# kehanxuuu/vspg-pbrt-v4

Hardware: AMD Instinct MI355X
Metric: Mpaths/sec on 1920x1080 homogeneous fog; relMSE vs CPU ref at equal spp (higher is better)
Workload: dtype f32; 1 GPU; fog-box 1920x1080, guidedvolpathvspg vspguiding=true (primary-ray VSP; App. F options), 1 spp per step per GPU, independent sampler seed 0, maxdepth 5

## Files before the change

### vspg-pbrt-v4_amd/csrc/vspg_capi.hip

```cpp
#include <hip/hip_runtime.h>
#include <dlfcn.h>

#include <cmath>
#include <cstdio>
#include <cstdlib>
#include <cstring>
#include <string>
#include <type_traits>
#include <vector>
#include <algorithm>

#include "vspg_path.h"
#include "vspg_wg_kernel.h"
#include "vspg_guided_wg.h"
#include "vspg_wg3.h"
#include "vspg_trace.h"
#include "vspg_wavefront.h"
#include "vspg_wf_launch.h"
#include "vspg_film_error.h"
#include "vspg_film_resolve.h"
#include "vspg_kernel_choice.h"
#ifdef VSPG_SINGLE_TU
#include "vspg_wf_grid.hip"
#include "vspg_wf_nvdb.hip"
// ... 1880 lines not shown
            float kd = in.Kd[k];
            kd = kd < 0 ? 0 : (kd > 1 ? 1 : kd);
            q.Kd[k] = kd;
            q.Le[k] = in.Le[k];
            lobes = lobes || kd != 0;
            light = light || in.Le[k] != 0;
        }
        q.two_sided = in.two_sided;
        q.is_light = light;
        q.has_lobes = lobes;
        q.flags = surf_flags_of(in.material, in.medium_interface);
        auto single_axis = [](const float *v) {
            int nz = 0, ax = -1;
            for (int k = 0; k < 3; ++k)
                if (v[k] != 0) { nz++; ax = k; }
            return nz == 1 ? ax : -1;
        };
        int an = single_axis(q.n), a1 = single_axis(q.e1), a2 = single_axis(q.e2);
        IsectRec &rec = D->irec[i];
        memset(&rec, 0, sizeof rec);
        if (an >= 0 && a1 >= 0 && a2 >= 0 && an != a1 && an != a2 && a1 != a2 && std::fabs(q.n[an]) == 1.0f) {
            rec.kind = 1;
            rec.axes = an | (a1 << 2) | (a2 << 4);
            rec.f[0] = q.n[an]; rec.f[1] = q.p00[an]; rec.f[2] = q.p00[a1]; rec.f[3] = q.p00[a2];
            rec.f[4] = q.e1[a1]; rec.f[5] = q.e2[a2]; rec.f[6] = q.inv_l1; rec.f[7] = q.inv_l2;
        } else {
            rec.kind = 0;
            for (int k = 0; k < 3; ++k) { rec.f[k] = q.n[k]; rec.f[3 + k] = q.p00[k]; rec.f[6 + k] = q.e1[k]; rec.f[9 + k] = q.e2[k]; }
            rec.f[12] = q.inv_l1; rec.f[13] = q.inv_l2;
        }
        if (light) D->light_quads[D->n_lights++] = i;
    }
    D->n_inf = sc.n_infinite_lights;
    for (int i = 0; i < sc.n_infinite_lights && i < VSPG_MAX_INFINITE_LIGHTS; ++i) {
        D->inf_type[i] = sc.infinite_lights[i].type;
        for (int k = 0; k < 3; ++k) { D->inf_L[i][k] = sc.infinite_lights[i].L[k]; D->inf_w[i][k] = sc.infinite_lights[i].w_light[k]; }
    }
    {
        float lo[3] = {kInf, kInf, kInf}, hi[3] = {-kInf, -kInf, -kInf};
        auto grow = [&](const float *q) { for (int k = 0; k < 3; ++k) { lo[k] = q[k] < lo[k] ? q[k] : lo[k]; hi[k] = q[k] > hi[k] ? q[k] : hi[k]; } };
        for (int i = 0; i < D->n_quads; ++i) { grow(D->quads[i].p00); grow(D->quads[i].p10); grow(D->quads[i].p01); grow(D->quads[i].p11); }
        for (int i = 0; i < sc.n_triangles && sc.tri_p; ++i) {
            DTri T;
            if (derive_triangle(sc.tri_p + 9 * (size_t)i, nullptr, i, &T)) { grow(T.p0); grow(T.p1); grow(T.p2); }
        }
        for (int i = 0; i < sc.n_spheres; ++i) {
            const float *m = sc.spheres[i].render_from_object, rr = sc.spheres[i].radius;
            for (int c = 0; c < 8; ++c) {
// ... 1979 lines not shown
```

### vspg-pbrt-v4_amd/csrc/vspg_device.h

```cpp
#pragma once
#include <hip/hip_runtime.h>
#include <stdint.h>

#include "../../include/vspg.h"
#include "vspg_arith.h"
#include "vspg_libm.h"

#define VDEV __device__ __forceinline__
#ifdef VSPG_WF_DEBUG
__device__ unsigned int g_dbg_err[8];
#define VSPG_DBG_CHECK(cond, bit) do { if (!(cond)) atomicOr(&g_dbg_err[0], 1u << (bit)); } while (0)
#else
#define VSPG_DBG_CHECK(cond, bit)
#endif
#ifdef VSPG_NOINLINE_LEAVES
#define VLEAF __device__ __attribute__((noinline))
#else
#define VLEAF __device__ __forceinline__
#endif

VSPG_NS_BEGIN

#ifdef VSPG_PROFILE
enum { PS_INTERSECT = 0, PS_HASHRNG, PS_DIST_GUIDED, PS_DIST_PLAIN, PS_SURF_PRE, PS_NEE, PS_NEE_TR, PS_VOL_SAMPLE,
// ... 403 lines not shown
    uint32_t r = ui + ((uint32_t)((int32_t)(ui ^ os) >> 31) | 1u);
    r = (ui << 1) == 0u ? (os | 1u) : r;
    const bool keep = !__builtin_islessgreater(off, 0.f) || (ui ^ os) == 0x7f800000u;
    return b2f(keep ? ui : r);
}
VDEV V3 offset_ray_origin(P3i pi, V3 n, V3 w) {
    float d = dot(vabs(n), pi.err());
    V3 offset = n * d;
    if (dot(w, n) < 0) offset = -offset;
    V3 po = pi.mid() + offset;
    return V3{offset_axis(po.x, offset.x), offset_axis(po.y, offset.y), offset_axis(po.z, offset.z)};
}

#define VSPG_GLOBAL_AS __attribute__((address_space(1)))
struct DQuad {
    float p00[3], p10[3], p01[3], p11[3], e1[3], e2[3];
    float n[3], dpdu_n[3], perr[3];
    float inv_l1, inv_l2, area;
    float Kd[3], Le[3];
    int32_t two_sided, is_light, has_lobes;
    int32_t flags;
};
enum { SURF_INTERFACE = 1, SURF_IFACE_SHIFT = 1 };
struct IsectRec {
    float f[14];
    int32_t kind;
    int32_t axes;
};
struct DField {
    int32_t n_nodes, n_regions;
    const VspgKdNode *nodes;
    const VspgFieldRegion *regions;
    const float *aux;
    const float4 *lobes;
};
constexpr int kMaxLights = VSPG_MAX_QUADS + VSPG_MAX_INFINITE_LIGHTS;
struct DLightNode {
    float bmin[3], bmax[3], w[3];
    float phi, cosTheta_o, cosTheta_e;
    int32_t twoSided;
    uint32_t child_or_light;
    int32_t is_leaf;
};
struct DLightSampler {
    int32_t mode;
    int32_t n_nodes, n_inf, n_alias;
    DLightNode nodes[2 * kMaxLights];
    int32_t inf_light[VSPG_MAX_INFINITE_LIGHTS];
    uint32_t bit_trail[kMaxLights];
    float alias_p[kMaxLights], alias_q[kMaxLights];
    int32_t alias_i[kMaxLights];
// ... 101 lines not shown
                            : k < 13 ? S.sigma_t[k - 10] : S.sigma_n_raw[k - 13];
    }
}
VDEV const DQuad &quad_at(int i) { return s_scene_quads[i]; }
VDEV const DQuad &light_quad_at(int lightIndex) { return s_scene_quads[s_scene_light_quads[lightIndex]]; }

struct Isect {
    bool hit;
    float t;
    int quad;
    V3 p, n;
};
VDEV bool is_tri(int prim) { return prim <= -2; }
VDEV int tri_of(int prim) { return -2 - prim; }
constexpr int kSpherePrim = 32;
static_assert(VSPG_MAX_QUADS <= kSpherePrim, "rectangle indices lie below the first sphere primitive");
VDEV bool is_sphere(int prim) { return prim >= kSpherePrim; }
VDEV int sphere_of(int prim) { return prim - kSpherePrim; }

VDEV bool beyond(float num, float denom, float tMax) {
    return __builtin_fabsf(num) > tMax * __builtin_fabsf(denom) * 1.000001f;
}
VDEV float comp(V3 v, int axis) { return axis == 0 ? v.x : (axis == 1 ? v.y : v.z); }
VDEV bool rect_hit_uv(const IsectRec &r, V3 o, V3 d, float tMax, float *tHit, float *uHit, float *vHit) {
    float num, denom, u, v, t;
    if (r.kind == 1) {
        const int a = r.axes & 3, ua = (r.axes >> 2) & 3, va = (r.axes >> 4) & 3;
        denom = r.f[0] * comp(d, a);
        num = r.f[0] * (r.f[1] - comp(o, a));
        bool cand = (num > 0 && denom > 0) || (num < 0 && denom < 0);
        if (!cand) return false;
        if (beyond(num, denom, tMax)) return false;
        t = num / denom;
        if (!(t > 0) || !(t < tMax)) return false;
        float pu = comp(o, ua) + comp(d, ua) * t, pv = comp(o, va) + comp(d, va) * t;
        u = ((pu - r.f[2]) * r.f[4]) * r.f[6];
        v = ((pv - r.f[3]) * r.f[5]) * r.f[7];
    } else {
        V3 n = V3{r.f[0], r.f[1], r.f[2]}, p00 = V3{r.f[3], r.f[4], r.f[5]};
        denom = dot(n, d);
        num = dot(n, p00 - o);
        bool cand = (num > 0 && denom > 0) || (num < 0 && denom < 0);
        if (!cand) return false;
        if (beyond(num, denom, tMax)) return false;
        t = num / denom;
        if (!(t > 0) || !(t < tMax)) return false;
        V3 p = o + d * t;
        V3 rel = p - p00;
        u = dot(rel, V3{r.f[6], r.f[7], r.f[8]}) * r.f[12];
        v = dot(rel, V3{r.f[9], r.f[10], r.f[11]}) * r.f[13];
    }
    if (u < 0 || u > 1 || v < 0 || v > 1) return false;
    *tHit = t;
    *uHit = u;
    *vHit = v;
    return true;
}
VDEV bool quad_hit_uv(const DQuad &q, V3 o, V3 d, float tMax, float *tHit, float *uHit, float *vHit) {
    V3 n = ld3(q.n), p00 = ld3(q.p00);
    float denom = dot(n, d);
    float num = dot(n, p00 - o);
    bool cand = (num > 0 && denom > 0) || (num < 0 && denom < 0);
    if (!cand) return false;
    float t = num / denom;
    if (!(t > 0) || !(t < tMax)) return false;
    V3 p = o + d * t;
    V3 rel = p - p00;
    float u = dot(rel, ld3(q.e1)) * q.inv_l1;
    float v = dot(rel, ld3(q.e2)) * q.inv_l2;
    if (u < 0 || u > 1 || v < 0 || v > 1) return false;
    *tHit = t;
    *uHit = u;
    *vHit = v;
// ... 251 lines not shown
        pv[k] = (row[0] * x + row[1] * y) + (row[2] * z + row[3]);
        const float ea = g3 * (__builtin_fabsf(row[0] * x) + __builtin_fabsf(row[1] * y) + __builtin_fabsf(row[2] * z) + __builtin_fabsf(row[3]));
        pe[k] = exact ? ea : (g3 + 1) * (__builtin_fabsf(row[0]) * ex + __builtin_fabsf(row[1]) * ey + __builtin_fabsf(row[2]) * ez) + ea;
    }
    r.pi = p3i_from_err(V3{pv[0], pv[1], pv[2]}, V3{pe[0], pe[1], pe[2]});
    const float *mi = S.mi;
    r.n = normalize(V3{mi[0] * no.x + mi[4] * no.y + mi[8] * no.z, mi[1] * no.x + mi[5] * no.y + mi[9] * no.z, mi[2] * no.x + mi[6] * no.y + mi[10] * no.z});
    if (WITH_DPDU) {
        const float *m = S.m;
        r.dpdu_n = normalize(V3{m[0] * dpdu.x + m[1] * dpdu.y + m[2] * dpdu.z, m[4] * dpdu.x + m[5] * dpdu.y + m[6] * dpdu.z, m[8] * dpdu.x + m[9] * dpdu.y + m[10] * dpdu.z});
    } else {
        r.dpdu_n = mk(0, 0, 0);
    }
    return r;
}

template <bool FULL = true>
VLEAF Isect scene_intersect(const DScene &S, V3 o, V3 d, float tMax) {
    Isect best;
    best.hit = false;
    best.t = tMax;
    best.quad = 0;
    float bu = 0, bv = 0;
    for (int i = 0; i < S.n_quads; ++i) {
        float t, u, v;
        if (rect_hit_uv(S.irec[i], o, d, best.t, &t, &u, &v)) {
            best.hit = true;
            best.t = t;
            best.quad = i;
            bu = u;
            bv = v;
        }
    }
    const DQuad &q = quad_at(best.quad);
    best.p = quad_point(q, bu, bv);
    best.n = ld3(q.n);
    if (FULL && S.n_tris > 0) {
        int tp = 0;
        TriHit h;
        if (bvh_closest(S, o, d, best.t, &tp, &h)) {
            const DTri &T = S.tris[tp];
            best.hit = true;
            best.t = h.t;
            best.quad = -2 - tp;
            best.p = V3{h.b0, h.b1, h.b2};
            best.n = V3{T.nx, T.ny, T.nz};
        }
    }
    if (FULL && S.n_spheres > 0) {
        for (int i = 0; i < S.n_spheres; ++i) {
            float t;
            V3 pObj;
            if (sphere_intersect(S.spheres[i], o, d, tMax, &t, &pObj) && t < best.t) {
                best.hit = true;
                best.t = t;
                best.quad = kSpherePrim + i;
                best.p = pObj;
                best.n = sphere_interaction<false>(S.spheres[i], pObj).n;
            }
        }
    }
    return best;
}
template <bool FULL = true>
VLEAF bool scene_intersect_any(const DScene &S, V3 o, V3 d, float tMax) {
    bool any = false;
    for (int i = 0; i < S.n_quads; ++i) {
        float t, u, v;
        any = any || rect_hit_uv(S.irec[i], o, d, tMax, &t, &u, &v);
    }
    if (FULL && S.n_tris > 0 && !any) any = bvh_any(S, o, d, tMax);
    if (FULL && S.n_spheres > 0 && !any) {
        for (int i = 0; i < S.n_spheres; ++i) {
            float t;
            V3 pObj;
            any = any || sphere_intersect(S.spheres[i], o, d, tMax, &t, &pObj);
        }
    }
    return any;
}
VDEV int surf_flags(const DScene &S, int prim) {
    if (is_tri(prim)) return S.tris[tri_of(prim)].flags;
    if (is_sphere(prim)) return S.spheres[sphere_of(prim)].flags;
    return quad_at(prim).flags;
}
VDEV P3i tri_pi(const DTri &T, V3 b) {
    const V3 p0 = ld3(T.p0), p1 = ld3(T.p1), p2 = ld3(T.p2);
    const V3 p = p0 * b.x + p1 * b.y + p2 * b.z;
    const V3 s = vabs(p0 * b.x) + vabs(p1 * b.y) + vabs(p2 * b.z);
    constexpr float g7 = (7 * kMachineEps) / (1 - 7 * kMachineEps);
    return p3i_from_err(p, V3{g7 * s.x, g7 * s.y, g7 * s.z});
}
// ... 647 lines not shown
```

### vspg-pbrt-v4_amd/csrc/vspg_wg3.h

```cpp
#pragma once
#include <type_traits>

#include "vspg_guided_wg.h"
#include "vspg_path.h"
#include "vspg_wg_kernel.h"

VSPG_NS_BEGIN

enum { Q_VV = 0, Q_VS = 1, Q_A = 2, Q_F = 3, Q_COUNT = 4 };
enum { QC_RES = 0, QC_COM = 1, QC_HEAD = 2, QC_STRIDE = 4 };
enum { W3_BUSY_S = Q_COUNT * QC_STRIDE, W3_BUSY_V, W3_EXH, W3_LIVE, W3_COUNT };
enum { W3_OLD = Q_VV * QC_STRIDE + 3, W3_SUSP_LO = Q_VS * QC_STRIDE + 3, W3_SUSP_HI = Q_A * QC_STRIDE + 3 };
constexpr unsigned kCarryDrainBit = 0x80000000u;
enum { W3_NONE = 0, W3_VERTEX = 1, W3_SEGMENT = 2, W3_FRESH = 3, W3_EXIT = 4 };
constexpr unsigned kRestartBit = 0x8000u;

VDEV float isg_code(const IsgSample &isg) {
    if (!isg.valid) return 0.f;
    const float q = isg.vsp_used >= 0.f ? isg.vsp_used : 0.5f;
    return isg.surface_event ? -q : q;
}
__device__ __forceinline__ void resolve_sample(float4 s, float4 *film_px, float *isg_px) {
    const Spec L = Spec{s.x, s.y, s.z};
    film_add_sample_rmw(film_px, L);
    IsgSample isg;
    isg.valid = s.w != 0.f;
    isg.surface_event = s.w < 0.f;
    isg.vsp_used = __builtin_fabsf(s.w);
    isg_add_sample_rmw(isg_px, L, isg);
}
template <class T>
__device__ __forceinline__ T w3_at_use(T v) {
    asm volatile("" : "+s"(v));
    return v;
}
__device__ __forceinline__ int w3_lane() {
    int l = (int)(threadIdx.x & 63u);
    asm volatile("" : "+v"(l));
    return l;
}
constexpr float kCarrySentinel = 2.f;
__device__ __forceinline__ bool carry_sentinel(float w) { return w > 1.f; }
template <class LY, int NP> constexpr int kWg3ImagePool = LY::COUNT * NP;
template <class LY, int NP> constexpr int kWg3ImageWords = LY::COUNT * NP + Q_COUNT * NP / 2;
template <class LY, int NP> constexpr int kWg3ImageStride = kWg3ImageWords<LY, NP> + 32;
static_assert(W3_COUNT <= 32, "the image's queue words");

constexpr int kWg3Heads = 8, kWg3HeadSetBytes = kWg3Heads * 128;
__device__ __forceinline__ void reset_sibling_head(unsigned int *work_head) {
    if (blockIdx.x == 0 && threadIdx.x == 0) *reinterpret_cast<unsigned int *>(reinterpret_cast<uintptr_t>(work_head) ^ 4u) = 0u;
}

typedef unsigned int w3_u32x4 __attribute__((ext_vector_type(4)));
typedef const volatile __attribute__((address_space(3))) w3_u32x4 *w3_lds_v4;
template <int NP>
VDEV void ring_push_all(int dq, unsigned entry, unsigned short (*ring)[NP], unsigned int *s_w) {
    const int lane = w3_lane();
    const unsigned long long m0 = __ballot(dq == 0), m1 = __ballot(dq == 1), m2 = __ballot(dq == 2), m3 = __ballot(dq == 3);
    const unsigned n0 = (unsigned)__popcll(m0), n1 = (unsigned)__popcll(m1), n2 = (unsigned)__popcll(m2), n3 = (unsigned)__popcll(m3);
    const unsigned myn = lane == 0 ? n0 : lane == 1 ? n1 : lane == 2 ? n2 : n3;
    unsigned base = 0;
    if (lane < Q_COUNT && myn > 0u) base = atomicAdd(s_w + lane * QC_STRIDE + QC_RES, myn);
    const unsigned b0 = (unsigned)__builtin_amdgcn_readlane((int)base, 0), b1 = (unsigned)__builtin_amdgcn_readlane((int)base, 1);
// ... 31 lines not shown
struct W3Timeline {
    unsigned long long *rec, t0;
    unsigned phase;
    __device__ __forceinline__ bool mine() const { return (threadIdx.x & 63u) == 0u && blockIdx.x < (unsigned)W3T_MAX_BLOCKS; }
    __device__ __forceinline__ W3Timeline() : rec(&g_w3_timeline[blockIdx.x % W3T_MAX_BLOCKS][(threadIdx.x >> 6) & 7u][0]), t0(0), phase(0) { stamp(W3T_BEGIN); }
    __device__ __forceinline__ void stamp(int i) { const unsigned long long t = __builtin_amdgcn_s_memrealtime(); if (mine()) rec[i] = t; }
    __device__ __forceinline__ void enter(unsigned p, int i) { if (phase < p) { phase = p; stamp(i); } }
    __device__ __forceinline__ void chunk_begin() { t0 = __builtin_amdgcn_s_memrealtime(); }
    __device__ __forceinline__ void chunk_end(unsigned kind, unsigned lanes) {
        const unsigned long long t1 = __builtin_amdgcn_s_memrealtime();
        if (mine()) {
            unsigned long long *r = rec + W3T_SUMS + (phase * 3u + kind) * 3u;
            atomicAdd(r, 1ull); atomicAdd(r + 1, (unsigned long long)lanes); atomicAdd(r + 2, t1 - t0);
        }
    }
};
#define VSPG_W3T(x) x
#else
#define VSPG_W3T(x)
#endif

template <class Medium, bool GUIDED, int NP, int kWgBlock, int kWgWavesPerSimd, bool TRAIN, bool WINDOW, bool CARRY = false>
__device__ __forceinline__ void wg3_render(
    const DScene *__restrict__ Sp, float4 *__restrict__ film, float *__restrict__ isg_stats, const float *__restrict__ vsp_buf,
    int vsp_ready, int wave_end, int first_sample, int single_sample, PcgJump jump, unsigned int tiles_magic,
    unsigned int *__restrict__ work_head, const float4 *__restrict__ prev_samples,
    float4 *__restrict__ wave_samples, unsigned long long *__restrict__ counters, TrainArgs train, const PixelWindow win,
    const unsigned int *__restrict__ resume = nullptr, unsigned int *__restrict__ suspend = nullptr) {
    static_assert(!CARRY || (!TRAIN && !GUIDED), "CARRY serves the unguided one-sample launches");
    vsp_ready = w3_at_use(vsp_ready), wave_end = w3_at_use(wave_end), first_sample = w3_at_use(first_sample);
    single_sample = w3_at_use(single_sample);
    const DScene &S = *Sp;
    const int W = S.xres, H = S.yres;
    const int tilesX = WINDOW ? win_tiles_x(win) : (W + 7) >> 3, tilesY = WINDOW ? win_tiles_y(win) : (H + 7) >> 3;
    const unsigned n_tiles = CARRY && w3_at_use(suspend) == nullptr ? 0u : (unsigned)(tilesX * tilesY);
    const auto in_launch = [&](int px, int py) {
        if constexpr (WINDOW) return win_has(win, px, py);
        else return px < W && py < H;
    };
    const int lane = threadIdx.x & 63;
    const int sample_step = S.shard_count > 1 ? S.shard_count : 1;
    if (blockIdx.x == 0 && threadIdx.x < (unsigned)kWg3Heads)
        reinterpret_cast<unsigned int *>(reinterpret_cast<uintptr_t>(work_head) ^ (uintptr_t)kWg3HeadSetBytes)[threadIdx.x * 32u] = 0u;
    unsigned wseg = blockIdx.x % (unsigned)kWg3Heads, wtried = 0u;

    constexpr bool FULL = !Medium::kSimpleScene;
    static_assert(!FULL || !GUIDED, "the workgroup kernel's guided vertex (vspg_guided_wg.h) is built for rectangle scenes");
    static_assert(NP < (int)kRestartBit, "a ring entry is the slot plus the restart bit");
    using LY = PoolLayout<GUIDED, Medium::kGrey, TRAIN, FULL>;
    constexpr int NF = LY::COUNT;
    static_assert(!TRAIN || GUIDED, "segment recording belongs to the guided instantiations");
    static_assert(Medium::kSingleSegment, "k_render_wave_wg3 serves homogeneous media (grid media: the wavefront pipeline)");
    __shared__ float s_pool[NF * NP];
    __shared__ unsigned short s_ring[Q_COUNT][NP];
    __shared__ __attribute__((aligned(16))) unsigned int s_w[W3_COUNT];
    const Pool P{s_pool, NP};
    const Medium medium = MediumMaker<Medium>::make(S, nullptr);
    float *glds = nullptr;
    if constexpr (GUIDED && kKdLdsNodes > 0) {
        __shared__ VspgKdNode s_kd[2][kKdLdsNodes > 0 ? kKdLdsNodes : 1];
        for (int f = 0; f < 2; ++f) {
            const int nl = S.field[f].n_nodes < kKdLdsNodes ? S.field[f].n_nodes : kKdLdsNodes;
            for (int i = threadIdx.x; i < nl; i += kWgBlock) s_kd[f][i] = S.field[f].nodes[i];
        }
        glds = reinterpret_cast<float *>(&s_kd[0][0]);
    }
    __shared__ unsigned int s_counters[CNT_COUNT];
    struct LaneCounters : PathCounters { uint32_t paths; VDEV void path() { paths++; } };
    using Rec = typename std::conditional<TRAIN, PathRecorder, NullRecorder>::type;
    typename std::conditional<GUIDED, WaveCountersT<Rec>, LaneCounters>::type pc = [&] {
        if constexpr (GUIDED) { WaveCountersT<Rec> c; c.c = s_counters; return c; }
        else { LaneCounters c; c.segments = c.volume_scatters = c.surface_hits = c.density_queries = c.shadow_rays = c.shadow_queries = c.paths = 0; return c; }
    }();
    const auto rec_bind = [&](int pxy) {
        if constexpr (TRAIN) {
            const unsigned px = (unsigned)pxy & 0xffffu, py = (unsigned)pxy >> 16;
            const unsigned tcol = WINDOW ? (px >> 3) - (unsigned)win_tile_x0(win) : px >> 3, trow = WINDOW ? (py >> 3) - (unsigned)win_tile_y0(win) : py >> 3;
            const unsigned item = (trow * (unsigned)tilesX + tcol) * 64u + ((py & 7u) << 3) + (px & 7u);
            pc.rec.base = train.segbuf + item;
            pc.rec.stride = (int)train.n_items;
            pc.rec.max_seg = train_rec_capacity(S.prm.maxdepth);
            return item;
        } else {
            (void)pxy;
            return 0u;
        }
    };

    stage_scene_lds(S);
    if (threadIdx.x < CNT_COUNT) s_counters[threadIdx.x] = 0;
    constexpr int kImgPool = kWg3ImagePool<LY, NP>, kImgWords = kWg3ImageWords<LY, NP>, kImgStride = kWg3ImageStride<LY, NP>;
    bool resumed = false;
    if constexpr (CARRY) {
        const unsigned int *const img = resume + (size_t)blockIdx.x * kImgStride;
        resumed = resume != nullptr && img[kImgWords + W3_LIVE] != 0u;
        if (resumed) {
            unsigned int *const pool32 = reinterpret_cast<unsigned int *>(s_pool);
#pragma unroll 8
            for (int i = threadIdx.x; i < kImgPool; i += kWgBlock) pool32[i] = img[i];
            unsigned short *const ring16 = &s_ring[0][0];
#pragma unroll 3
            for (int i = threadIdx.x; i < Q_COUNT * NP / 2; i += kWgBlock) {
                const unsigned v = img[kImgPool + i];
                ring16[2 * i] = (unsigned short)(v & 0xffffu);
                ring16[2 * i + 1] = (unsigned short)(v >> 16);
            }
            if (threadIdx.x < W3_COUNT) s_w[threadIdx.x] = img[kImgWords + threadIdx.x];
            __syncthreads();
            if (threadIdx.x < Q_COUNT) {
                const unsigned h = s_w[threadIdx.x * QC_STRIDE + QC_HEAD], n = s_w[threadIdx.x * QC_STRIDE + QC_COM] - h, h2 = h % (unsigned)NP;
                s_w[threadIdx.x * QC_STRIDE + QC_HEAD] = h2;
                s_w[threadIdx.x * QC_STRIDE + QC_RES] = h2 + n;
                s_w[threadIdx.x * QC_STRIDE + QC_COM] = h2 + n;
            }
            if (threadIdx.x == 0) {
                s_w[W3_OLD] = s_w[W3_LIVE];
                s_w[W3_EXH] = 0u;
                s_w[W3_BUSY_S] = 0u;
                s_w[W3_BUSY_V] = 0u;
            }
        }
    }
    if (!resumed) {
        if (threadIdx.x < W3_COUNT) s_w[threadIdx.x] = 0;
        for (int i = threadIdx.x; i < NP; i += kWgBlock) s_ring[Q_F][i] = (unsigned short)i;
        __syncthreads();
        if (threadIdx.x == 0) {
            s_w[Q_F * QC_STRIDE + QC_RES] = NP; s_w[Q_F * QC_STRIDE + QC_COM] = NP;
        }
    }
    if constexpr (CARRY) {
        __syncthreads();
        if (threadIdx.x == 0) {
            if (suspend == nullptr) { s_w[W3_EXH] = 1u; s_w[W3_OLD] |= kCarryDrainBit; }
            s_w[W3_SUSP_LO] = (unsigned)reinterpret_cast<uintptr_t>(suspend);
            s_w[W3_SUSP_HI] = (unsigned)(reinterpret_cast<uintptr_t>(suspend) >> 32);
        }
    }
    __syncthreads();

    auto emit = [&](int pxy, Spec Lraw, const IsgSample &isg, bool old) {
        const Spec L = finish_radiance(Lraw);
        const size_t pidx = (size_t)((unsigned)pxy >> 16) * W + (pxy & 0xffff);
        if (CARRY && old && w3_at_use(first_sample) >= 0) {
            resolve_sample(make_float4(L.r, L.g, L.b, isg_code(isg)), film + pidx, isg_stats + pidx * VSPG_ISG_STATS);
        } else if (w3_at_use(single_sample)) {
            wave_samples[pidx] = make_float4(L.r, L.g, L.b, isg_code(isg));
        } else {
            film_add_sample(film + pidx, L);
            isg_add_sample_atomic(isg_stats + pidx * VSPG_ISG_STATS, L, isg);
        }
    };

    VSPG_PROF(PS_WG_TOTAL);
    VSPG_PROF_ACC(prof_decide, PS_WG_R);
    VSPG_PROF_ACC(prof_idle, PS_WG_BAR_A);
    unsigned idle_polls = 0;
    VSPG_W3T(W3Timeline tl);
    while (true) {
        VSPG_PROF_ACC_BEGIN(prof_decide);
        VSPG_PROF_ACC_BEGIN(prof_idle);
        unsigned kind = W3_NONE, pos0 = 0, n0 = 0, pos1 = 0, n1 = 0, q0 = Q_VV, tile = 0;
        unsigned fresh_entry = 0;
        {
            const auto U = [](unsigned v) { return (unsigned)__builtin_amdgcn_readfirstlane((int)v); };
            const w3_lds_v4 qw = (w3_lds_v4)(s_w);
            const w3_u32x4 wVV = qw[Q_VV], wVS = qw[Q_VS], wA = qw[Q_A], wF = qw[Q_F], wM = qw[Q_COUNT];
            const unsigned hVV = U(wVV.z), hVS = U(wVS.z), hA = U(wA.z), hF = U(wF.z);
            const unsigned busyS = U(wM.x), busyV = U(wM.y), live = U(wM.w);
            const unsigned old_word = CARRY ? U(wVV.w) : 1u;
            const bool exh = U(wM.z) != 0u;
            VSPG_W3T(if (exh) tl.enter(2u, W3T_EXH));
            const auto avail = [&](w3_u32x4 q, unsigned head) {
// ... 18 lines not shown
                } else {
                    bump(W3_BUSY_V, -1);
                }
            };
            const auto claim_segment = [&]() {
                bump(W3_BUSY_S, 1);
                const unsigned na = (unsigned)(aA < 64 ? aA : 64);
                if (claim(Q_A, hA, na)) { kind = W3_SEGMENT; pos0 = hA; n0 = na; }
                else bump(W3_BUSY_S, -1);
            };
            const int aV = aVV + aVS;
            if (CARRY && exh && old_word == 0u) kind = W3_EXIT;
            else if (aVV >= 64) claim_vertex(aVV, hVV, Q_VV, 0, hVS, Q_VS);
            else if (aVS >= 64) claim_vertex(aVS, hVS, Q_VS, 0, hVV, Q_VV);
            else if (aA >= 64) claim_segment();
            else if (aF >= 64) {
                bump(W3_BUSY_S, 1);
                bump(W3_LIVE, 64);
                if (claim(Q_F, hF, 64u)) {
                    kind = W3_FRESH; pos0 = hF; n0 = 64u;
                    __builtin_amdgcn_fence(__ATOMIC_ACQUIRE, "workgroup");
                    fresh_entry = s_ring[Q_F][(hF + (unsigned)lane) % (unsigned)NP];
                    tile = n_tiles;
                    while (wtried < (unsigned)kWg3Heads) {
                        unsigned c = 0xffffffffu;
                        if (w3_lane() == 0 && __hip_atomic_load(work_head + wseg * 32u, __ATOMIC_RELAXED, __HIP_MEMORY_SCOPE_AGENT) * (unsigned)kWg3Heads + wseg < n_tiles)
                            c = atomicAdd(work_head + wseg * 32u, 1u);
                        c = U(c);
                        if (c != 0xffffffffu && c * (unsigned)kWg3Heads + wseg < n_tiles) {
                            tile = c * (unsigned)kWg3Heads + wseg;
                            break;
                        }
                        wseg = (wseg + 1u) % (unsigned)kWg3Heads;
                        ++wtried;
                    }
                } else {
                    bump(W3_LIVE, -64);
                    bump(W3_BUSY_S, -1);
                }
            } else if (aV >= 64 || (aV > 0 && busyS == 0u)) {
                if (aVV >= aVS) claim_vertex(aVV, hVV, Q_VV, aVS, hVS, Q_VS);
                else claim_vertex(aVS, hVS, Q_VS, aVV, hVV, Q_VV);
            } else if (aA > 0 && busyV == 0u) {
                claim_segment();
            } else if (exh && live == 0u) {
                kind = W3_EXIT;
// ... 76 lines not shown
                freed = true;
            } else if ((unsigned)lane < n0) {
                const unsigned e = fresh ? fresh_entry : s_ring[Q_A][(pos0 + (unsigned)lane) % (unsigned)NP];
                slot = (int)(e & (kRestartBit - 1u));
                const bool primary = fresh || (e & kRestartBit) != 0u;
                Sampler sampler;
                PathState st;
                IsgSample isg;
                int ch = 0, pxy = 0;
                Vertex vx;
                bool alive = false, valid = true;
                int seg = LI_END;
                if (primary) {
                    int px, py, smp;
                    if (fresh) {
                        unsigned ty = w3_at_use(tilesX) == 1 ? tile : __umulhi(tile, tiles_magic);
                        unsigned tx = tile - ty * (unsigned)tilesX;
                        while (tx >= (unsigned)tilesX) { tx -= (unsigned)tilesX; ty++; }
                        if constexpr (WINDOW) { tx += (unsigned)win_tile_x0(win); ty += (unsigned)win_tile_y0(win); }
                        px = (int)(tx * 8u + ((unsigned)lane & 7u));
                        py = (int)(ty * 8u + ((unsigned)lane >> 3));
                        pxy = px | (py << 16);
                        smp = first_sample;
                        if (w3_at_use(prev_samples) != nullptr && in_launch(px, py)) {
                            const size_t pidx = (size_t)py * W + px;
                            const float4 parked = prev_samples[pidx];
                            if (!(CARRY && carry_sentinel(parked.w)))
                                resolve_sample(parked, film + pidx, isg_stats + pidx * VSPG_ISG_STATS);
                        }
                    } else {
                        pxy = P.i(LY::PIXEL, slot);
                        smp = P.i(LY::SAMPLE, slot);
                        px = pxy & 0xffff;
                        py = (int)((unsigned)pxy >> 16);
                    }
                    valid = in_launch(px, py) && smp < wave_end;
                    if (valid) {
                        if (w3_at_use(single_sample))
                            start_path(S, vsp_buf, w3_at_use(vsp_ready), px, py, jump, sampler, st, &ch, isg);
                        else
                            start_path(S, vsp_buf, w3_at_use(vsp_ready), px, py, smp, sampler, st, &ch, isg);
                        P.i(LY::PIXEL, slot) = pxy;
                        P.i(LY::SAMPLE, slot) = smp;
                        if constexpr (TRAIN) { (void)rec_bind(pxy); pc.rec.reset(); }
                        seg = li_segment_a<Medium, GUIDED, SEG_PRIMARY>(S, medium, vsp_buf, w3_at_use(vsp_ready), px, py, st, ch, sampler,
                                                                        isg, pc, vx);
                        alive = seg != LI_END;
                        if (alive) {
                            pool_store_full<GUIDED, Medium::kGrey, FULL>(P, slot, st, sampler, ch, isg, FL_LIVE | (seg == LI_VERTEX && vx.volume ? (uint32_t)FL_VX_VOLUME : 0u));
                            if (seg == LI_VERTEX) pool_store_vertex<GUIDED, Medium::kGrey>(P, slot, vx);
                            if constexpr (TRAIN) pool_store_rec<LY>(P, slot, pc.rec);
// ... 32 lines not shown
                    freed = !restart;
                }
            }
            ring_push_all<NP>(toVV ? Q_VV : toVS ? Q_VS : (toA || restart) ? Q_A : (freed ? Q_F : -1), (unsigned)slot | (restart ? kRestartBit : 0u), s_ring, s_w);
            const unsigned n_freed = (unsigned)__popcll(__ballot(freed));
            const unsigned n_old = CARRY ? (unsigned)__popcll(__ballot(old_done)) : 0u;
            if (w3_lane() == 0) {
                if (CARRY && n_old) atomicSub(s_w + W3_OLD, n_old);
                if (fresh && !tile_ok) atomicExch(s_w + W3_EXH, 1u);
                if (n_freed) atomicSub(s_w + W3_LIVE, n_freed);
                atomicSub(s_w + W3_BUSY_S, 1u);
            }
            VSPG_W3T(tl.chunk_end(fresh ? 2u : 1u, tile_ok ? n0 : 0u));
        }
    }
    VSPG_W3T(tl.stamp(W3T_EXIT));
    if constexpr (!GUIDED) {
        atomicAdd(&s_counters[CNT_PATHS], pc.paths); atomicAdd(&s_counters[CNT_SEGMENTS], pc.segments);
        atomicAdd(&s_counters[CNT_VOLUME_SCATTERS], pc.volume_scatters); atomicAdd(&s_counters[CNT_SURFACE_HITS], pc.surface_hits);
        atomicAdd(&s_counters[CNT_DENSITY_QUERIES], pc.density_queries); atomicAdd(&s_counters[CNT_SHADOW_RAYS], pc.shadow_rays);
        atomicAdd(&s_counters[CNT_SHADOW_QUERIES], pc.shadow_queries);
    }
    __syncthreads();
    if (threadIdx.x < CNT_COUNT) atomicAdd(&counters[threadIdx.x], (unsigned long long)s_counters[threadIdx.x]);
    if constexpr (CARRY) {
        unsigned int *const susp = reinterpret_cast<unsigned int *>((uintptr_t)s_w[W3_SUSP_LO] | ((uintptr_t)s_w[W3_SUSP_HI] << 32));
        if (susp != nullptr) {
            unsigned int *const img = susp + (size_t)blockIdx.x * kImgStride;
            if (threadIdx.x < W3_COUNT) img[kImgWords + threadIdx.x] = s_w[threadIdx.x];
            if (s_w[W3_LIVE] != 0u) {
                const unsigned int *const pool32 = reinterpret_cast<const unsigned int *>(s_pool);
                for (int i = threadIdx.x; i < kImgPool; i += kWgBlock) img[i] = pool32[i];
                const unsigned short *const ring16 = &s_ring[0][0];
                for (int i = threadIdx.x; i < Q_COUNT * NP / 2; i += kWgBlock) img[kImgPool + i] = (unsigned)ring16[2 * i] | ((unsigned)ring16[2 * i + 1] << 16);
                for (int q = 0; q < Q_F; ++q) {
                    const unsigned h = s_w[q * QC_STRIDE + QC_HEAD], n = s_w[q * QC_STRIDE + QC_COM] - h;
                    for (unsigned i = threadIdx.x; i < n && i < (unsigned)NP; i += kWgBlock) {
                        const int pxy = P.i(LY::PIXEL, (int)(s_ring[q][(h + i) % (unsigned)NP] & (kRestartBit - 1u)) % NP);
                        const unsigned px = (unsigned)pxy & 0xffffu, py = (unsigned)pxy >> 16;
                        if (in_launch((int)px, (int)py)) wave_samples[(size_t)py * W + px].w = kCarrySentinel;
                    }
                }
            }
        }
    }
}

template <class Medium, bool GUIDED, int NP, int kWgBlock, int kWgWavesPerSimd, bool TRAIN = false>
__global__ __launch_bounds__(kWgBlock, kWgWavesPerSimd) void k_render_wave_wg3(
    const DScene *__restrict__ Sp, float4 *__restrict__ film, float *__restrict__ isg_stats, const float *__restrict__ vsp_buf,
    int vsp_ready, int wave_end, int first_sample, int single_sample, PcgJump jump, unsigned int tiles_magic,
    unsigned int *__restrict__ work_head, const float4 *__restrict__ prev_samples,
    float4 *__restrict__ wave_samples, unsigned long long *__restrict__ counters, TrainArgs train = TrainArgs{nullptr, nullptr, nullptr, nullptr, 0, 0}) {
    wg3_render<Medium, GUIDED, NP, kWgBlock, kWgWavesPerSimd, TRAIN, false>(Sp, film, isg_stats, vsp_buf, vsp_ready, wave_end, first_sample, single_sample, jump,
                                                                            tiles_magic, work_head, prev_samples, wave_samples, counters, train, PixelWindow{0, 0, 0, 0});
}
template <class Medium, bool GUIDED, int NP, int kWgBlock, int kWgWavesPerSimd, bool TRAIN = false>
__global__ __launch_bounds__(kWgBlock, kWgWavesPerSimd) void k_render_wave_wg3_window(
    const DScene *__restrict__ Sp, float4 *__restrict__ film, float *__restrict__ isg_stats, const float *__restrict__ vsp_buf,
    int vsp_ready, int wave_end, int first_sample, int single_sample, PcgJump jump, unsigned int tiles_magic,
    unsigned int *__restrict__ work_head, const float4 *__restrict__ prev_samples,
    float4 *__restrict__ wave_samples, unsigned long long *__restrict__ counters, TrainArgs train, PixelWindow win) {
    wg3_render<Medium, GUIDED, NP, kWgBlock, kWgWavesPerSimd, TRAIN, true>(Sp, film, isg_stats, vsp_buf, vsp_ready, wave_end, first_sample, single_sample, jump,
                                                                           tiles_magic, work_head, prev_samples, wave_samples, counters, train, win);
}

template <class Medium, bool GUIDED, int NP, int kWgBlock, int kWgWavesPerSimd, bool WINDOW>
__global__ __launch_bounds__(kWgBlock, kWgWavesPerSimd) void k_render_wave_wg3_carry(
    const DScene *__restrict__ Sp, float4 *__restrict__ film, float *__restrict__ isg_stats, const float *__restrict__ vsp_buf,
    int vsp_ready, int wave_end, int first_sample, int single_sample, PcgJump jump, unsigned int tiles_magic,
    unsigned int *__restrict__ work_head, const float4 *__restrict__ prev_samples,
    float4 *__restrict__ wave_samples, unsigned long long *__restrict__ counters, PixelWindow win,
    const unsigned int *__restrict__ resume, unsigned int *__restrict__ suspend) {
    wg3_render<Medium, GUIDED, NP, kWgBlock, kWgWavesPerSimd, false, WINDOW, true>(Sp, film, isg_stats, vsp_buf, vsp_ready, wave_end, first_sample, single_sample, jump,
                                                                                   tiles_magic, work_head, prev_samples, wave_samples, counters,
                                                                                   TrainArgs{nullptr, nullptr, nullptr, nullptr, 0, 0}, win, resume, suspend);
}

#ifndef VSPG_WG_WAVES
#define VSPG_WG_WAVES 4
#endif
#ifndef VSPG_WG_BLOCK
#define VSPG_WG_BLOCK 512
#endif
struct Wg3Launch {
    const DScene *dscene;
    float4 *film;
    float *isg_stats;
    const float *vsp;
    int vsp_ready, wave_end, first_sample, single_sample;
    PcgJump jump;
    unsigned int tiles_magic;
    unsigned int *work_head;
    const float4 *ws_prev;
    float4 *ws_out;
    unsigned long long *counters;
    unsigned int blocks;
    hipStream_t stream;
// ... 44 lines not shown
```

Before: 3630 Mpaths/s.

## Split intersection records into 32-byte halves, prefetch heads, reload kernargs at use

Reorders IsectRec into a 32-byte head {kind, axes, f[0..5]} and a 32-byte tail, loaded as 8-wide scalar vectors. The next rectangle's head is prefetched while the current one is tested, and the tail is fetched only once the plane test passes. Separately, kernel pointers (film, isg_stats, wave_samples, counters, prev_samples, work_head) are re-read from the kernarg segment where they are used instead of being held live, to reduce SGPR pressure. The ring load/store becomes 32-bit copies instead of split 16-bit writes. The risks are extra scalar loads and reliance on inline-asm tricks to steer codegen.

```diff
diff --git a/vspg-pbrt-v4_amd/csrc/vspg_capi.hip b/vspg-pbrt-v4_amd/csrc/vspg_capi.hip
--- a/vspg-pbrt-v4_amd/csrc/vspg_capi.hip
+++ b/vspg-pbrt-v4_amd/csrc/vspg_capi.hip
@@ -1926,8 +1926,9 @@
         if (an >= 0 && a1 >= 0 && a2 >= 0 && an != a1 && an != a2 && a1 != a2 && std::fabs(q.n[an]) == 1.0f) {
             rec.kind = 1;
             rec.axes = an | (a1 << 2) | (a2 << 4);
-            rec.f[0] = q.n[an]; rec.f[1] = q.p00[an]; rec.f[2] = q.p00[a1]; rec.f[3] = q.p00[a2];
-            rec.f[4] = q.e1[a1]; rec.f[5] = q.e2[a2]; rec.f[6] = q.inv_l1; rec.f[7] = q.inv_l2;
+            rec.f[0] = q.n[an]; rec.f[1] = q.p00[an];
+            rec.f[6] = q.p00[a1]; rec.f[7] = q.p00[a2];
+            rec.f[8] = q.e1[a1]; rec.f[9] = q.e2[a2]; rec.f[10] = q.inv_l1; rec.f[11] = q.inv_l2;
         } else {
             rec.kind = 0;
             for (int k = 0; k < 3; ++k) { rec.f[k] = q.n[k]; rec.f[3 + k] = q.p00[k]; rec.f[6 + k] = q.e1[k]; rec.f[9 + k] = q.e2[k]; }
diff --git a/vspg-pbrt-v4_amd/csrc/vspg_device.h b/vspg-pbrt-v4_amd/csrc/vspg_device.h
--- a/vspg-pbrt-v4_amd/csrc/vspg_device.h
+++ b/vspg-pbrt-v4_amd/csrc/vspg_device.h
@@ -449,11 +449,16 @@
     int32_t flags;
 };
 enum { SURF_INTERFACE = 1, SURF_IFACE_SHIFT = 1 };
-struct IsectRec {
-    float f[14];
+struct alignas(32) IsectRec {
     int32_t kind;
     int32_t axes;
-};
+    float f[14];
+};
+static_assert(sizeof(IsectRec) == 64 && alignof(IsectRec) == 32, "two 32-byte halves");
+static_assert(offsetof(IsectRec, kind) == 0 && offsetof(IsectRec, axes) == 4 && offsetof(IsectRec, f) == 8, "the head: {kind, axes, f[0..5]}");
+static_assert(offsetof(IsectRec, f) + 6 * sizeof(float) == 32, "the tail f[6..13] is the second half");
+typedef int32_t irec_i32x8 __attribute__((ext_vector_type(8)));
+typedef float irec_f32x8 __attribute__((ext_vector_type(8)));
 struct DField {
     int32_t n_nodes, n_regions;
     const VspgKdNode *nodes;
@@ -601,22 +606,37 @@
     return __builtin_fabsf(num) > tMax * __builtin_fabsf(denom) * 1.000001f;
 }
 VDEV float comp(V3 v, int axis) { return axis == 0 ? v.x : (axis == 1 ? v.y : v.z); }
-VDEV bool rect_hit_uv(const IsectRec &r, V3 o, V3 d, float tMax, float *tHit, float *uHit, float *vHit) {
+template <class T>
+VDEV T rect_half(const DScene &S, int i, uint32_t half) {
+    uint32_t off = (uint32_t)offsetof(DScene, irec) + (uint32_t)i * (uint32_t)sizeof(IsectRec) + half * 32u;
+    asm volatile("" : "+s"(off));
+    return *reinterpret_cast<const T *>(reinterpret_cast<const char *>(&S) + off);
+}
+VDEV irec_i32x8 rect_head(const DScene &S, int i) { return rect_half<irec_i32x8>(S, i, 0u); }
+VDEV irec_f32x8 rect_tail(const DScene &S, int i) { return rect_half<irec_f32x8>(S, i, 1u); }
+VDEV void rect_head_arrived(const irec_i32x8 h) {
+    const int32_t kind = h[0];
+    asm volatile("" : : "s"(kind));
+}
+VDEV bool rect_hit_uv(const DScene &S, int i, const irec_i32x8 h, V3 o, V3 d, float tMax, float *tHit, float *uHit, float *vHit) {
     float num, denom, u, v, t;
-    if (r.kind == 1) {
-        const int a = r.axes & 3, ua = (r.axes >> 2) & 3, va = (r.axes >> 4) & 3;
-        denom = r.f[0] * comp(d, a);
-        num = r.f[0] * (r.f[1] - comp(o, a));
+    const auto hf = [&](int k) { const int32_t w = h[2 + k]; return __builtin_bit_cast(float, w); };
+    if (h[0] == 1) {
+        const int axes = h[1];
+        const int a = axes & 3, ua = (axes >> 2) & 3, va = (axes >> 4) & 3;
+        denom = hf(0) * comp(d, a);
+        num = hf(0) * (hf(1) - comp(o, a));
         bool cand = (num > 0 && denom > 0) || (num < 0 && denom < 0);
         if (!cand) return false;
         if (beyond(num, denom, tMax)) return false;
         t = num / denom;
         if (!(t > 0) || !(t < tMax)) return false;
         float pu = comp(o, ua) + comp(d, ua) * t, pv = comp(o, va) + comp(d, va) * t;
-        u = ((pu - r.f[2]) * r.f[4]) * r.f[6];
-        v = ((pv - r.f[3]) * r.f[5]) * r.f[7];
+        const irec_f32x8 g = rect_tail(S, i);
+        u = ((pu - g[0]) * g[2]) * g[4];
+        v = ((pv - g[1]) * g[3]) * g[5];
     } else {
-        V3 n = V3{r.f[0], r.f[1], r.f[2]}, p00 = V3{r.f[3], r.f[4], r.f[5]};
+        V3 n = V3{hf(0), hf(1), hf(2)}, p00 = V3{hf(3), hf(4), hf(5)};
         denom = dot(n, d);
         num = dot(n, p00 - o);
         bool cand = (num > 0 && denom > 0) || (num < 0 && denom < 0);
@@ -626,8 +646,9 @@
         if (!(t > 0) || !(t < tMax)) return false;
         V3 p = o + d * t;
         V3 rel = p - p00;
-        u = dot(rel, V3{r.f[6], r.f[7], r.f[8]}) * r.f[12];
-        v = dot(rel, V3{r.f[9], r.f[10], r.f[11]}) * r.f[13];
+        const irec_f32x8 g = rect_tail(S, i);
+        u = dot(rel, V3{g[0], g[1], g[2]}) * g[6];
+        v = dot(rel, V3{g[3], g[4], g[5]}) * g[7];
     }
     if (u < 0 || u > 1 || v < 0 || v > 1) return false;
     *tHit = t;
@@ -925,9 +946,14 @@
     best.t = tMax;
     best.quad = 0;
     float bu = 0, bv = 0;
-    for (int i = 0; i < S.n_quads; ++i) {
+    const int nq = S.n_quads;
+    irec_i32x8 head = rect_head(S, 0);
+    for (int i = 0; i < nq; ++i) {
         float t, u, v;
-        if (rect_hit_uv(S.irec[i], o, d, best.t, &t, &u, &v)) {
+        const irec_i32x8 h = head;
+        rect_head_arrived(h);
+        head = rect_head(S, i + 1 < nq ? i + 1 : i);
+        if (rect_hit_uv(S, i, h, o, d, best.t, &t, &u, &v)) {
             best.hit = true;
             best.t = t;
             best.quad = i;
@@ -968,9 +994,14 @@
 template <bool FULL = true>
 VLEAF bool scene_intersect_any(const DScene &S, V3 o, V3 d, float tMax) {
     bool any = false;
-    for (int i = 0; i < S.n_quads; ++i) {
+    const int nq = S.n_quads;
+    irec_i32x8 head = rect_head(S, 0);
+    for (int i = 0; i < nq; ++i) {
         float t, u, v;
-        any = any || rect_hit_uv(S.irec[i], o, d, tMax, &t, &u, &v);
+        const irec_i32x8 h = head;
+        rect_head_arrived(h);
+        head = rect_head(S, i + 1 < nq ? i + 1 : i);
+        any = any || rect_hit_uv(S, i, h, o, d, tMax, &t, &u, &v);
     }
     if (FULL && S.n_tris > 0 && !any) any = bvh_any(S, o, d, tMax);
     if (FULL && S.n_spheres > 0 && !any) {
diff --git a/vspg-pbrt-v4_amd/csrc/vspg_wg3.h b/vspg-pbrt-v4_amd/csrc/vspg_wg3.h
--- a/vspg-pbrt-v4_amd/csrc/vspg_wg3.h
+++ b/vspg-pbrt-v4_amd/csrc/vspg_wg3.h
@@ -39,6 +39,38 @@
     asm volatile("" : "+v"(l));
     return l;
 }
+struct Wg3KernArgs {
+    const DScene *Sp;
+    float4 *film;
+    float *isg_stats;
+    const float *vsp_buf;
+    int vsp_ready, wave_end, first_sample, single_sample;
+    PcgJump jump;
+    unsigned int tiles_magic;
+    unsigned int *work_head;
+    const float4 *prev_samples;
+    float4 *wave_samples;
+    unsigned long long *counters;
+};
+template <class T>
+__device__ __forceinline__ T w3_karg(uint32_t offset) {
+    asm volatile("" : "+s"(offset));
+    typedef const __attribute__((address_space(4))) char *karg_bytes;
+    typedef const __attribute__((address_space(4))) T *karg_T;
+    return *(karg_T)((karg_bytes)__builtin_amdgcn_kernarg_segment_ptr() + offset);
+}
+#define VSPG_W3_KARG(field) w3_karg<decltype(Wg3KernArgs::field)>((uint32_t)offsetof(Wg3KernArgs, field))
+struct Wg3FilmArgs {
+    float4 *film;
+    float *isg_stats;
+};
+static_assert(offsetof(Wg3KernArgs, isg_stats) == offsetof(Wg3KernArgs, film) + sizeof(float4 *) && sizeof(Wg3FilmArgs) == 16, "neighbours");
+typedef unsigned long long w3_u64x2 __attribute__((ext_vector_type(2), aligned(8)));
+__device__ __forceinline__ Wg3FilmArgs w3_film_args() {
+    const w3_u64x2 v = w3_karg<w3_u64x2>((uint32_t)offsetof(Wg3KernArgs, film));
+    return Wg3FilmArgs{reinterpret_cast<float4 *>(v.x), reinterpret_cast<float *>(v.y)};
+}
+
 constexpr float kCarrySentinel = 2.f;
 __device__ __forceinline__ bool carry_sentinel(float w) { return w > 1.f; }
 template <class LY, int NP> constexpr int kWg3ImagePool = LY::COUNT * NP;
@@ -116,10 +148,9 @@
 
 template <class Medium, bool GUIDED, int NP, int kWgBlock, int kWgWavesPerSimd, bool TRAIN, bool WINDOW, bool CARRY = false>
 __device__ __forceinline__ void wg3_render(
-    const DScene *__restrict__ Sp, float4 *__restrict__ film, float *__restrict__ isg_stats, const float *__restrict__ vsp_buf,
+    const DScene *__restrict__ Sp, const float *__restrict__ vsp_buf,
     int vsp_ready, int wave_end, int first_sample, int single_sample, PcgJump jump, unsigned int tiles_magic,
-    unsigned int *__restrict__ work_head, const float4 *__restrict__ prev_samples,
-    float4 *__restrict__ wave_samples, unsigned long long *__restrict__ counters, TrainArgs train, const PixelWindow win,
+    unsigned int *__restrict__ work_head, TrainArgs train, const PixelWindow win,
     const unsigned int *__restrict__ resume = nullptr, unsigned int *__restrict__ suspend = nullptr) {
     static_assert(!CARRY || (!TRAIN && !GUIDED), "CARRY serves the unguided one-sample launches");
     vsp_ready = w3_at_use(vsp_ready), wave_end = w3_at_use(wave_end), first_sample = w3_at_use(first_sample);
@@ -146,7 +177,7 @@
     static_assert(!TRAIN || GUIDED, "segment recording belongs to the guided instantiations");
     static_assert(Medium::kSingleSegment, "k_render_wave_wg3 serves homogeneous media (grid media: the wavefront pipeline)");
     __shared__ float s_pool[NF * NP];
-    __shared__ unsigned short s_ring[Q_COUNT][NP];
+    __shared__ __attribute__((aligned(4))) unsigned short s_ring[Q_COUNT][NP];
     __shared__ __attribute__((aligned(16))) unsigned int s_w[W3_COUNT];
     const Pool P{s_pool, NP};
     const Medium medium = MediumMaker<Medium>::make(S, nullptr);
@@ -192,13 +223,9 @@
             unsigned int *const pool32 = reinterpret_cast<unsigned int *>(s_pool);
 #pragma unroll 8
             for (int i = threadIdx.x; i < kImgPool; i += kWgBlock) pool32[i] = img[i];
-            unsigned short *const ring16 = &s_ring[0][0];
+            unsigned int *const ring32 = reinterpret_cast<unsigned int *>(&s_ring[0][0]);
 #pragma unroll 3
-            for (int i = threadIdx.x; i < Q_COUNT * NP / 2; i += kWgBlock) {
-                const unsigned v = img[kImgPool + i];
-                ring16[2 * i] = (unsigned short)(v & 0xffffu);
-                ring16[2 * i + 1] = (unsigned short)(v >> 16);
-            }
+            for (int i = threadIdx.x; i < Q_COUNT * NP / 2; i += kWgBlock) ring32[i] = img[kImgPool + i];
             if (threadIdx.x < W3_COUNT) s_w[threadIdx.x] = img[kImgWords + threadIdx.x];
             __syncthreads();
             if (threadIdx.x < Q_COUNT) {
@@ -235,14 +262,16 @@
 
     auto emit = [&](int pxy, Spec Lraw, const IsgSample &isg, bool old) {
         const Spec L = finish_radiance(Lraw);
-        const size_t pidx = (size_t)((unsigned)pxy >> 16) * W + (pxy & 0xffff);
+                const size_t pidx = (size_t)((unsigned)pxy >> 16) * W + (pxy & 0xffff);
         if (CARRY && old && w3_at_use(first_sample) >= 0) {
-            resolve_sample(make_float4(L.r, L.g, L.b, isg_code(isg)), film + pidx, isg_stats + pidx * VSPG_ISG_STATS);
+            const Wg3FilmArgs fa = w3_film_args();
+            resolve_sample(make_float4(L.r, L.g, L.b, isg_code(isg)), fa.film + pidx, fa.isg_stats + pidx * VSPG_ISG_STATS);
         } else if (w3_at_use(single_sample)) {
-            wave_samples[pidx] = make_float4(L.r, L.g, L.b, isg_code(isg));
+            VSPG_W3_KARG(wave_samples)[pidx] = make_float4(L.r, L.g, L.b, isg_code(isg));
         } else {
-            film_add_sample(film + pidx, L);
-            isg_add_sample_atomic(isg_stats + pidx * VSPG_ISG_STATS, L, isg);
+            const Wg3FilmArgs fa = w3_film_args();
+            film_add_sample(fa.film + pidx, L);
+            isg_add_sample_atomic(fa.isg_stats + pidx * VSPG_ISG_STATS, L, isg);
         }
     };
 
@@ -307,6 +336,7 @@
                     __builtin_amdgcn_fence(__ATOMIC_ACQUIRE, "workgroup");
                     fresh_entry = s_ring[Q_F][(hF + (unsigned)lane) % (unsigned)NP];
                     tile = n_tiles;
+                    unsigned int *const work_head = VSPG_W3_KARG(work_head);
                     while (wtried < (unsigned)kWg3Heads) {
                         unsigned c = 0xffffffffu;
                         if (w3_lane() == 0 && __hip_atomic_load(work_head + wseg * 32u, __ATOMIC_RELAXED, __HIP_MEMORY_SCOPE_AGENT) * (unsigned)kWg3Heads + wseg < n_tiles)
@@ -429,11 +459,14 @@
                         py = (int)(ty * 8u + ((unsigned)lane >> 3));
                         pxy = px | (py << 16);
                         smp = first_sample;
-                        if (w3_at_use(prev_samples) != nullptr && in_launch(px, py)) {
-                            const size_t pidx = (size_t)py * W + px;
+                        const float4 *const prev_samples = VSPG_W3_KARG(prev_samples);
+                        if (prev_samples != nullptr && in_launch(px, py)) {
+                                                        const size_t pidx = (size_t)py * W + px;
                             const float4 parked = prev_samples[pidx];
-                            if (!(CARRY && carry_sentinel(parked.w)))
-                                resolve_sample(parked, film + pidx, isg_stats + pidx * VSPG_ISG_STATS);
+                            if (!(CARRY && carry_sentinel(parked.w))) {
+                                const Wg3FilmArgs fa = w3_film_args();
+                                resolve_sample(parked, fa.film + pidx, fa.isg_stats + pidx * VSPG_ISG_STATS);
+                            }
                         }
                     } else {
                         pxy = P.i(LY::PIXEL, slot);
@@ -512,7 +545,9 @@
         atomicAdd(&s_counters[CNT_SHADOW_QUERIES], pc.shadow_queries);
     }
     __syncthreads();
-    if (threadIdx.x < CNT_COUNT) atomicAdd(&counters[threadIdx.x], (unsigned long long)s_counters[threadIdx.x]);
+    unsigned tid = threadIdx.x;
+    asm volatile("" : "+v"(tid));
+    if (tid < (unsigned)CNT_COUNT) atomicAdd(&VSPG_W3_KARG(counters)[tid], (unsigned long long)s_counters[tid]);
     if constexpr (CARRY) {
         unsigned int *const susp = reinterpret_cast<unsigned int *>((uintptr_t)s_w[W3_SUSP_LO] | ((uintptr_t)s_w[W3_SUSP_HI] << 32));
         if (susp != nullptr) {
@@ -521,14 +556,14 @@
             if (s_w[W3_LIVE] != 0u) {
                 const unsigned int *const pool32 = reinterpret_cast<const unsigned int *>(s_pool);
                 for (int i = threadIdx.x; i < kImgPool; i += kWgBlock) img[i] = pool32[i];
-                const unsigned short *const ring16 = &s_ring[0][0];
-                for (int i = threadIdx.x; i < Q_COUNT * NP / 2; i += kWgBlock) img[kImgPool + i] = (unsigned)ring16[2 * i] | ((unsigned)ring16[2 * i + 1] << 16);
+                const unsigned int *const ring32 = reinterpret_cast<const unsigned int *>(&s_ring[0][0]);
+                for (int i = threadIdx.x; i < Q_COUNT * NP / 2; i += kWgBlock) img[kImgPool + i] = ring32[i];
                 for (int q = 0; q < Q_F; ++q) {
                     const unsigned h = s_w[q * QC_STRIDE + QC_HEAD], n = s_w[q * QC_STRIDE + QC_COM] - h;
                     for (unsigned i = threadIdx.x; i < n && i < (unsigned)NP; i += kWgBlock) {
                         const int pxy = P.i(LY::PIXEL, (int)(s_ring[q][(h + i) % (unsigned)NP] & (kRestartBit - 1u)) % NP);
                         const unsigned px = (unsigned)pxy & 0xffffu, py = (unsigned)pxy >> 16;
-                        if (in_launch((int)px, (int)py)) wave_samples[(size_t)py * W + px].w = kCarrySentinel;
+                        if (in_launch((int)px, (int)py)) VSPG_W3_KARG(wave_samples)[(size_t)py * W + px].w = kCarrySentinel;
                     }
                 }
             }
@@ -542,8 +577,8 @@
     int vsp_ready, int wave_end, int first_sample, int single_sample, PcgJump jump, unsigned int tiles_magic,
     unsigned int *__restrict__ work_head, const float4 *__restrict__ prev_samples,
     float4 *__restrict__ wave_samples, unsigned long long *__restrict__ counters, TrainArgs train = TrainArgs{nullptr, nullptr, nullptr, nullptr, 0, 0}) {
-    wg3_render<Medium, GUIDED, NP, kWgBlock, kWgWavesPerSimd, TRAIN, false>(Sp, film, isg_stats, vsp_buf, vsp_ready, wave_end, first_sample, single_sample, jump,
-                                                                            tiles_magic, work_head, prev_samples, wave_samples, counters, train, PixelWindow{0, 0, 0, 0});
+    wg3_render<Medium, GUIDED, NP, kWgBlock, kWgWavesPerSimd, TRAIN, false>(Sp, vsp_buf, vsp_ready, wave_end, first_sample, single_sample, jump,
+                                                                            tiles_magic, work_head, train, PixelWindow{0, 0, 0, 0});
 }
 template <class Medium, bool GUIDED, int NP, int kWgBlock, int kWgWavesPerSimd, bool TRAIN = false>
 __global__ __launch_bounds__(kWgBlock, kWgWavesPerSimd) void k_render_wave_wg3_window(
@@ -551,8 +586,8 @@
     int vsp_ready, int wave_end, int first_sample, int single_sample, PcgJump jump, unsigned int tiles_magic,
     unsigned int *__restrict__ work_head, const float4 *__restrict__ prev_samples,
     float4 *__restrict__ wave_samples, unsigned long long *__restrict__ counters, TrainArgs train, PixelWindow win) {
-    wg3_render<Medium, GUIDED, NP, kWgBlock, kWgWavesPerSimd, TRAIN, true>(Sp, film, isg_stats, vsp_buf, vsp_ready, wave_end, first_sample, single_sample, jump,
-                                                                           tiles_magic, work_head, prev_samples, wave_samples, counters, train, win);
+    wg3_render<Medium, GUIDED, NP, kWgBlock, kWgWavesPerSimd, TRAIN, true>(Sp, vsp_buf, vsp_ready, wave_end, first_sample, single_sample, jump,
+                                                                           tiles_magic, work_head, train, win);
 }
 
 template <class Medium, bool GUIDED, int NP, int kWgBlock, int kWgWavesPerSimd, bool WINDOW>
@@ -562,8 +597,8 @@
     unsigned int *__restrict__ work_head, const float4 *__restrict__ prev_samples,
     float4 *__restrict__ wave_samples, unsigned long long *__restrict__ counters, PixelWindow win,
     const unsigned int *__restrict__ resume, unsigned int *__restrict__ suspend) {
-    wg3_render<Medium, GUIDED, NP, kWgBlock, kWgWavesPerSimd, false, WINDOW, true>(Sp, film, isg_stats, vsp_buf, vsp_ready, wave_end, first_sample, single_sample, jump,
-                                                                                   tiles_magic, work_head, prev_samples, wave_samples, counters,
+    wg3_render<Medium, GUIDED, NP, kWgBlock, kWgWavesPerSimd, false, WINDOW, true>(Sp, vsp_buf, vsp_ready, wave_end, first_sample, single_sample, jump,
+                                                                                   tiles_magic, work_head,
                                                                                    TrainArgs{nullptr, nullptr, nullptr, nullptr, 0, 0}, win, resume, suspend);
 }
 
```

New measurement: 3622 Mpaths/s. No clear change (-0.2%).
